# xingyizhou/CenterNet

Measured on AMD Instinct MI355X. Metric: images/sec whole-node, 512x512 ctdet, higher is better.
Workload: dtype f32s; 1 GPU; ctdet resdcn_18 512x512, batch 32 per GPU (BASELINE configs[1]), network + fused sigmoid/peak-NMS/top-K decode, K=100; global_batch=32, parallelism=image-sharded x1

## Files before the change

centernet_amd/csrc/cn_conv.hip:

```cpp
#include "cn_internal.h"
#include "cn_tuning.h"
#include <type_traits>

#ifndef CN_IGEMM_F32S_SETS
#define CN_IGEMM_F32S_SETS 1
#endif

namespace {

constexpr int NT = 256;
constexpr int BK = 32;
constexpr int LDT = BK + 4;

enum { A_DENSE = 0, A_STEM = 1, A_DCN = 2, A_DCN_PAD = 3 };
constexpr int STEM_KMAX = 512;

struct IgemmArgs {
    const void *x;
    const void *w;
    const float *bias;
    const float *scale;
    const float *shift;
    const void *residual;
    void *y;
// ... 596 lines not shown
            }
        }
    } else {
        const int OHW = a.OH * a.OW;
#pragma unroll
        for (int i = 0; i < MB; ++i) {
            const int off = rowoff[wm * TM + i * 32 + l31];
            const int b = off >= 0 ? off / OHW : 0;
            const int rem = off - b * OHW;
#pragma unroll
            for (int j = 0; j < NB; ++j) {
#pragma unroll
                for (int r = 0; r < 16; ++r) {
                    const int n = n0 + wn * TN + j * 32 + (r & 3) + 8 * (r >> 2) + 4 * lh;
                    if (off >= 0 && n < a.Cout) {
                        const float bs = a.bias ? a.bias[n] : 0.f;
                        const float sc = a.scale ? a.scale[n] : 1.f;
                        const float sf = a.shift ? a.shift[n] : 0.f;
                        float v = (acc[i][j][r] + bs) * sc + sf;
                        if (a.relu) v = fmaxf(v, 0.f);
                        reinterpret_cast<float *>(a.y)[((size_t)b * a.Cout + n) * OHW + rem] = v;
                    }
                }
            }
        }
    }
    if constexpr (SPLIT) {
        if (a.range) {
            if (!OUT_NCHW && !a.out_plain && a.ksplit <= 1) cn_rng_commit(a.range, 0, rng_out);
            if (DCN || a.in_plain) cn_rng_commit(a.range, 1, rng_in);
        }
    }
}

template <int BM, int BN, int WM, int AMODE, bool OUT_NCHW, int NBUF>
constexpr size_t igemm_lds_bytes()
{
    constexpr size_t tiles = (size_t)NBUF * (BM + BN) * LDT;
    constexpr size_t cs = OUT_NCHW ? 0 : (size_t)(BM / WM) * (BN + 4);
    return (tiles > cs ? tiles : cs) * 4 + BM * 4 +
           ((AMODE == A_DCN || AMODE == A_DCN_PAD) ? (size_t)9 * BM * (4 * 4 + 4 * 4 + 4) : 0) +
           (AMODE == A_STEM ? (size_t)STEM_KMAX * 8 : 0);
}

template <typename T, int BM, int BN, int WM, int WN, int AMODE, bool OUT_NCHW, int NBUF>
int launch_igemm_n(const IgemmArgs &a, hipStream_t st)
{
    constexpr size_t lds = igemm_lds_bytes<BM, BN, WM, AMODE, OUT_NCHW, NBUF>();
    CN_SET_MAX_LDS_ONCE((igemm_kernel<T, BM, BN, WM, WN, AMODE, OUT_NCHW, NBUF>), lds);
    dim3 grid(cn_cdiv(a.M, BM), cn_cdiv(a.Cout, BN), a.zparity ? 4 : (a.ksplit > 1 ? a.ksplit : 1));
    IgemmArgs b = a;
    b.xcd_swizzle = (grid.x >= 16 && cn_knobs.swz != 2 && (AMODE == A_DCN || AMODE == A_DCN_PAD || cn_knobs.swz == 1)) ? 1 : 0;
    b.setprio = cn_knobs.setprio;
    b.dbgskip = cn_knobs.dbgskip;
    hipLaunchKernelGGL((igemm_kernel<T, BM, BN, WM, WN, AMODE, OUT_NCHW, NBUF>), grid, dim3(NT),
                       lds, st, b);
    CN_CHECK_LAUNCH();
    return CN_OK;
}

template <int BM, int BN, int WM, int WN, int AMODE, bool OUT_NCHW>
int launch_igemm_h(const IgemmArgs &a, hipStream_t st)
{
    static_assert(AMODE != A_DCN && AMODE != A_DCN_PAD, "fp16 DCN is not built");
    if (!OUT_NCHW && AMODE == A_DENSE && a.stride == 1)
        return launch_igemm_n<_Float16, BM, BN, WM, WN, AMODE, OUT_NCHW, 1>(a, st);
    return launch_igemm_n<_Float16, BM, BN, WM, WN, AMODE, OUT_NCHW, 2>(a, st);
}

template <int BM, int BN, int WM, int WN, int AMODE, bool OUT_NCHW>
int launch_igemm_s(const IgemmArgs &a, hipStream_t st)
{
    static_assert(AMODE != A_STEM, "the stem stays on the fp32 kernel");
    if (!OUT_NCHW && a.stride == 1 && cn_knobs.nbuf != 2)
        return launch_igemm_n<cn_f32s, BM, BN, WM, WN, AMODE, OUT_NCHW, 1>(a, st);
    return launch_igemm_n<cn_f32s, BM, BN, WM, WN, AMODE, OUT_NCHW, 2>(a, st);
}

template <int BM, int BN, int WM, int WN, int AMODE, bool OUT_NCHW>
int launch_igemm(const IgemmArgs &a, hipStream_t st)
{
    int nbuf = cn_knobs.nbuf ? cn_knobs.nbuf : (a.stride == 1 ? 1 : 2);
    if (AMODE == A_STEM || OUT_NCHW) nbuf = 2;
    if (nbuf == 1) {
        if constexpr (AMODE != A_STEM && !OUT_NCHW)
            return launch_igemm_n<float, BM, BN, WM, WN, AMODE, OUT_NCHW, 1>(a, st);
    }
    return launch_igemm_n<float, BM, BN, WM, WN, AMODE, OUT_NCHW, 2>(a, st);
}

template <int BM, int BN, int WM, int WN, int AMODE, bool OUT_NCHW>
int launch_igemm_t(int dtype, const IgemmArgs &a, hipStream_t st)
{
    if constexpr (AMODE != A_STEM) {
        if (dtype == CN_DTYPE_F32S) return launch_igemm_s<BM, BN, WM, WN, AMODE, OUT_NCHW>(a, st);
    }
    if constexpr (AMODE == A_DENSE || AMODE == A_STEM) {
        if (dtype == CN_DTYPE_F16) return launch_igemm_h<BM, BN, WM, WN, AMODE, OUT_NCHW>(a, st);
    }
    return launch_igemm<BM, BN, WM, WN, AMODE, OUT_NCHW>(a, st);
}

inline int cout_class(int Cout) { return Cout > 64 ? 2 : (Cout > 32 ? 1 : 0); }
template <int AMODE, bool OUT_NCHW>
int igemm_dispatch(int dtype, int cls, bool bm64, const IgemmArgs &a, hipStream_t st)
{
    constexpr bool DCN = AMODE == A_DCN || AMODE == A_DCN_PAD;
// ... 488 lines not shown
{
    if (cn_knobs.nosplit || cn_knobs.dcn_split == 1) return 1;
    if (cn_knobs.dcn_split == 3 || cn_knobs.dcn_split == 9) return cn_knobs.dcn_split;
    const long wgs = (long)cn_cdiv(B * H * W, 64) * cn_cdiv(Cout, Cout > 64 ? 128 : 64);
    if (wgs >= 1024) return 1;
    return wgs * 3 >= 600 ? 3 : 9;
}

extern "C" size_t cn_dcn_v2_forward_nhwc_workspace_bytes(int B, int Cin, int H, int W, int Cout)
{
    if (B <= 0 || Cin <= 0 || H <= 0 || W <= 0 || Cout <= 0) return 0;
    const int s = dcn_ksplit(B, H, W, Cout);
    return s > 1 ? (size_t)(s > 8 ? s : 8) * B * H * W * round_up(Cout, 32) * sizeof(float) : 0;
}

extern "C" int cn_dcn_v2_forward_nhwc_f32(const float *input_nhwc, const float *weight_packed,
                                          const float *bias, const float *offset_mask_nhwc,
                                          int om_pitch, const float *scale, const float *shift,
                                          float *output_nhwc, int B, int Cin, int H, int W,
                                          int Cout, int mask_sigmoid, int relu, void *workspace,
                                          size_t workspace_bytes, void *stream)
{
    return cn_dcn_v2_forward_nhwc(input_nhwc, weight_packed, bias, offset_mask_nhwc, om_pitch, scale,
                                  shift, output_nhwc, Cout, B, Cin, H, W, Cout, mask_sigmoid, relu,
                                  CN_DTYPE_F32, 0, nullptr, workspace, workspace_bytes, stream);
}

extern "C" int cn_dcn_v2_forward_nhwc(const float *input_nhwc, const void *weight_packed,
                                      const float *bias, const float *offset_mask_nhwc,
                                      int om_pitch, const float *scale, const float *shift,
                                      void *output_nhwc, int out_pitch, int B, int Cin, int H,
                                      int W, int Cout, int mask_sigmoid, int relu, int dtype,
                                      int flags, const cn_f32s_ctl *ctl, void *workspace,
                                      size_t workspace_bytes, void *stream)
{
    if (!input_nhwc || !weight_packed || !offset_mask_nhwc || !output_nhwc) return CN_ERR_NULL;
    if (B <= 0 || Cin <= 0 || H <= 0 || W <= 0 || Cout <= 0 || out_pitch < Cout) return CN_ERR_SHAPE;
    if (om_pitch < 27) return CN_ERR_SHAPE;
    if ((Cin & 3) != 0) return CN_ERR_UNSUPPORTED;
    const bool f32s = (dtype == CN_DTYPE_F32S);
    if (dtype != CN_DTYPE_F32 && !f32s) return CN_ERR_UNSUPPORTED;
    if (f32s && !(flags & CN_CONV_Y_PLAIN) && (out_pitch & 31)) return CN_ERR_UNSUPPORTED;
    if (!cn_aligned16(input_nhwc) || !cn_aligned16(weight_packed)) return CN_ERR_ALIGN;
    if (f32s && !(flags & CN_CONV_Y_PLAIN) && !aligned128(output_nhwc)) return CN_ERR_ALIGN;
    if ((long)B * H * W * (long)(Cin > out_pitch ? Cin : out_pitch) >= (1L << 30)) return CN_ERR_UNSUPPORTED;
    if (f32s && cn_knobs.dcn_form != 1) {
        const bool forced = cn_knobs.dcn_form >= 2;
        const bool ws_ok = workspace && cn_aligned16(workspace) && !cn_knobs.nosplit;
        int ks = 1;
        int rc = CN_ERR_UNSUPPORTED;
        const long tiles128 = (long)B * (H / 8) * (W / 16);
        const bool team_auto = cn_knobs.dcn_form == 0 && tiles128 >= 64 &&
                               ((cn_knobs.dcn_team == 1 && Cout <= 64) || cn_knobs.dcn_team >= 2);
        const bool wide_auto = cn_knobs.dcn_form == 0 && cn_knobs.dcn_wide && tiles128 >= 64 && (Cout & 127) == 0 && !cn_knobs.dbgskip;
        DcnWinCall c = {};
        c.x = input_nhwc; c.w = weight_packed; c.bias = bias; c.om = offset_mask_nhwc; c.om_pitch = om_pitch;
        c.scale = scale; c.shift = shift; c.y = output_nhwc; c.out_pitch = out_pitch;
        c.out_plain = (flags & CN_CONV_Y_PLAIN) ? 1 : 0;
        c.B = B; c.Cin = Cin; c.H = H; c.W = W; c.Cout = Cout; c.mask_sigmoid = mask_sigmoid; c.relu = relu;
        c.x_mul = (ctl && ctl->x_mul != 0.f) ? ctl->x_mul : 1.f;
        c.range = ctl ? ctl->range : nullptr;
        c.dbg = cn_knobs.dbgskip;
        c.partial = ws_ok ? (float *)workspace : nullptr;
        c.partial_bytes = ws_ok ? workspace_bytes : 0;
        hipStream_t st = (hipStream_t)stream;
        if (cn_knobs.dcn_form == 6 || cn_knobs.dcn_form == 7 || wide_auto)
            rc = cn_dcn_wide_f32s(c, cn_knobs.dcn_form == 7 ? 4 : 0, &ks, st);
        if (rc == CN_ERR_UNSUPPORTED && (cn_knobs.dcn_form == 4 || cn_knobs.dcn_form == 5 || team_auto))
            rc = cn_dcn_team_f32s(c, cn_knobs.dcn_form == 5 ? 2 : ((team_auto && cn_knobs.dcn_team == 3) ? 1 : 0), &ks, st);
        if (rc == CN_ERR_UNSUPPORTED && cn_knobs.dcn_form < 4)
            rc = cn_dcn_window_f32s(c, forced ? 1 : 192, &ks, st);
        if (rc == CN_OK && ks > 1) {
            IgemmArgs r = {};
            r.bias = bias; r.scale = scale; r.shift = shift; r.residual = nullptr; r.y = output_nhwc;
            set_ctl(r, ctl);
            r.B = B; r.H = H; r.W = W; r.Ho = H; r.Wo = W; r.Cout = Cout; r.out_pitch = out_pitch;
            r.out_plain = (flags & CN_CONV_Y_PLAIN) ? 1 : 0;
            r.OH = H; r.OW = W; r.oy_mul = 1; r.oy_add = 0; r.ox_mul = 1; r.ox_add = 0;
            r.relu = relu; r.M = B * H * W; r.cout_pad = round_up(Cout, 32);
            r.ksplit = ks; r.partial = (float *)workspace;
            return launch_splitk_reduce(CN_DTYPE_F32S, r, 4096, (hipStream_t)stream);
        }
        if (rc != CN_ERR_UNSUPPORTED) return rc;
    }
    IgemmArgs a = {};
    a.x = input_nhwc; a.w = weight_packed; a.bias = bias; a.scale = scale; a.shift = shift;
    a.residual = nullptr; a.y = output_nhwc; a.om = offset_mask_nhwc; a.om_pitch = om_pitch;
    a.mask_sigmoid = mask_sigmoid;
    set_ctl(a, ctl);
    a.B = B; a.H = H; a.W = W; a.Cin = Cin; a.Ho = H; a.Wo = W; a.Cout = Cout;
    a.KH = 3; a.KW = 3; a.stride = 1; a.pad_h = 1; a.pad_w = 1; a.dil = 1;
    a.in_pitch = Cin; a.out_pitch = out_pitch;
    a.in_plain = 1;
    a.out_plain = (flags & CN_CONV_Y_PLAIN) ? 1 : 0;
    a.OH = H; a.OW = W; a.oy_mul = 1; a.oy_add = 0; a.ox_mul = 1; a.ox_add = 0;
    a.relu = relu;
    a.M = B * H * W;
    a.cin_pad = round_up(Cin, 32);
    a.cout_pad = round_up(Cout, 32);
    a.nchunk = a.cin_pad / 32;
    a.KT = 9 * a.nchunk;
    a.vec_out = ((Cout & 3) == 0 && (out_pitch & 3) == 0 && cn_aligned16(output_nhwc)) ? 1 : 0;
    hipStream_t st = (hipStream_t)stream;
    a.tile2d = (cn_knobs.dcn_tile2d && (W & 7) == 0 && (H % (Cout > 32 ? 8 : 16)) == 0) ? 1 : 0;
    a.ksplit = 1;
    if (Cout > 32) {
        const int want = dcn_ksplit(B, H, W, Cout);
        const size_t need = (size_t)want * a.M * a.cout_pad * sizeof(float);
        if (want > 1 && workspace && workspace_bytes >= need && cn_aligned16(workspace)) {
            a.ksplit = want;
            a.partial = (float *)workspace;
        }
    }
    const int rc = (Cin & 31) ? igemm_dispatch<A_DCN_PAD, false>(dtype, cout_class(Cout), false, a, st)
                              : igemm_dispatch<A_DCN, false>(dtype, cout_class(Cout), false, a, st);
// ... 144 lines not shown
```

centernet_amd/csrc/cn_heads_at.hip:

```cpp
#include "cn_common.h"
#include "cn_internal.h"

namespace {

constexpr int HA_NT = 256;
constexpr int HA_CELLS = 16;
constexpr int HA_CC = 64;
constexpr int HA_ROW = 9 * HA_CC;
constexpr int HA_MAXN = 768;
constexpr int HA_MAXJ = 17;
constexpr int HA_MAXOUT = 2 + 2 * HA_MAXJ + 2;
enum { HA_CTDET = 0, HA_POSE = 1, HA_DDD = 2 };
constexpr int HA_PF = 4;
constexpr int HA_MAXGROUPS = 5;
constexpr int HA_GROUP_HEADS = 3;
constexpr int HA_DDD_OUT = 16;

struct HeadsAtGroup {
    const cn_f32x4 *w1;
    const float *b1, *w2, *b2;
    int n_heads;
    int cout[HA_GROUP_HEADS];
    int col[HA_GROUP_HEADS];
    int voff[HA_GROUP_HEADS];
};

struct HeadsAtArgs {
    const char *feat;
    const float *scores;
    const int32_t *inds, *clses;
    const cn_f32x4 *w1;
    const float *b1;
    const float *w2;
    const float *b2;
    float *dets;
    float *vals;
    float mul;
    int H, W, Cin, pitch, K, hidden, n_heads, N;
    int c0, c1;
    int out;
    int J;
    HeadsAtGroup grp[HA_MAXGROUPS];
    int D;
    int vals_out;
    int raw_depth;
    int half_group;
};

__device__ __forceinline__ void ha_ctdet_row(const HeadsAtArgs &a, size_t row, int ind, const float *o)
{
    float *d = a.dets + row * 6;
    const float score = a.scores[row];
    const float cls = (float)a.clses[row];
    if (ind < 0) {
        const float nan = __builtin_nanf("");
        d[0] = nan; d[1] = nan; d[2] = nan; d[3] = nan; d[4] = score; d[5] = cls;
        if (a.vals)
            for (int v = 0; v < a.out; ++v) a.vals[row * a.out + v] = nan;
        return;
    }
    const int yi = ind / a.W, xi = ind - yi * a.W;
    float xs = (float)xi, ys = (float)yi;
    if (a.n_heads > 1) {
        xs = xs + o[2];
        ys = ys + o[3];
    } else {
        xs = xs + 0.5f;
        ys = ys + 0.5f;
    }
    const float w = o[0];
    const float h = o[1];
    d[0] = xs - w / 2;
    d[1] = ys - h / 2;
    d[2] = xs + w / 2;
    d[3] = ys + h / 2;
    d[4] = score;
    d[5] = cls;
    if (a.vals)
        for (int v = 0; v < a.out; ++v) a.vals[row * a.out + v] = o[v];
}

__device__ __forceinline__ float ha_pose_col(const HeadsAtArgs &a, size_t row, int ind, const float *o, int col)
{
    const int D = 5 + 2 * a.J + 1;
    if (col == 4) return a.scores[row];
    if (col == D - 1) return (float)a.clses[row];
    if (ind < 0) return __builtin_nanf("");
    const int yi = ind / a.W, xi = ind - yi * a.W;
    if (col >= 5) {
        const int v = col - 5;
        return o[2 + v] + (float)((v & 1) ? yi : xi);
    }
    const bool isy = col & 1;
    float c = (float)(isy ? yi : xi);
    if (a.n_heads > 2) c = c + o[2 + 2 * a.J + (isy ? 1 : 0)];
    else c = c + 0.5f;
    const float half = o[isy ? 1 : 0] / 2;
    return col < 2 ? c - half : c + half;
}

template <bool F32S, int CT, int NS, int TASK = HA_CTDET>
__global__ __launch_bounds__(HA_NT) void decode_heads_at_cells_kernel(const HeadsAtArgs a)
{
    constexpr int CG = HA_CELLS / CT;
    constexpr int TPC = HA_NT / CG;
    static_assert(TPC % 64 == 0, "the lanes of a wave read one cell's patch");
    constexpr int HROW = NS * TPC > HA_ROW ? NS * TPC : HA_ROW;
    static_assert(NS * TPC <= HA_MAXN && HA_CELLS * HROW * 4 <= 48 * 1024, "static LDS");
    __shared__ __attribute__((aligned(16))) float lds[HA_CELLS * HROW];
    __shared__ int s_ind[HA_CELLS];
    __shared__ float s_out[HA_CELLS * (TASK == HA_POSE ? HA_MAXOUT : TASK == HA_DDD ? HA_DDD_OUT : 4)];

    const int tid = threadIdx.x;
    const int b = blockIdx.y;
    const int k0 = blockIdx.x * HA_CELLS;
    const int ncell = min(HA_CELLS, a.K - k0);
    const int HW = a.H * a.W;
    int N = a.N, out = a.out, hc0 = a.c0, hc1 = a.c1;
    const cn_f32x4 *w1 = a.w1;
    const float *b1 = a.b1, *w2 = a.w2, *b2 = a.b2;
    if constexpr (TASK == HA_DDD) {
        const HeadsAtGroup &g = a.grp[blockIdx.z];
        N = g.n_heads * a.hidden;
        hc0 = g.cout[0];
        hc1 = g.cout[1];
        out = hc0 + hc1 + g.cout[2];
        w1 = g.w1; b1 = g.b1; w2 = g.w2; b2 = g.b2;
    }

    if (tid < HA_CELLS) {
        int ind = -1;
        if (tid < ncell) {
            ind = a.inds[(size_t)b * a.K + k0 + tid];
            if ((uint32_t)ind >= (uint32_t)HW) ind = -1;
        }
        s_ind[tid] = ind;
    }

    const int nl = tid % TPC, cg = tid / TPC;
    float acc[NS][CT];
#pragma unroll
    for (int s = 0; s < NS; ++s)
#pragma unroll
        for (int i = 0; i < CT; ++i) acc[s][i] = 0.f;

    size_t kq_base = 0;
    for (int c0 = 0; c0 < a.Cin; c0 += HA_CC) {
        const int cc = min(HA_CC, a.Cin - c0);
        const int cq = cc >> 2;
        __syncthreads();
        for (int i = tid; i < HA_CELLS * 9 * cq; i += HA_NT) {
            const int q = i % cq, r = i / cq;
            const int tap = r % 9, cell = r / 9;
            const int ind = s_ind[cell];
            cn_f32x4 v = {0.f, 0.f, 0.f, 0.f};
            if (ind >= 0) {
                const int y = ind / a.W + tap / 3 - 1, x = ind % a.W + tap % 3 - 1;
                if ((unsigned)y < (unsigned)a.H && (unsigned)x < (unsigned)a.W) {
                    const size_t pix = ((size_t)b * a.H + y) * a.W + x;
                    if (F32S) {
                        v = cn_load4_f32s(a.feat, pix, a.pitch, c0 + 4 * q);
                        v *= a.mul;
                    } else {
                        v = *reinterpret_cast<const cn_f32x4 *>(a.feat + (pix * (size_t)a.pitch + c0 + 4 * q) * 4);
                    }
                }
            }
            *reinterpret_cast<cn_f32x4 *>(&lds[cell * HA_ROW + tap * cc + 4 * q]) = v;
        }
        __syncthreads();

        const int nkq = 9 * cq;
        const cn_f32x4 *wq = w1 + kq_base * N;
        cn_f32x4 wn[HA_PF][NS];
#pragma unroll
        for (int p = 0; p < HA_PF; ++p)
#pragma unroll
            for (int s = 0; s < NS; ++s) {
                const int n = nl + s * TPC;
                wn[p][s] = n < N ? wq[(size_t)p * N + n] : cn_f32x4{0.f, 0.f, 0.f, 0.f};
            }
        for (int kq = 0; kq < nkq; kq += HA_PF) {
            cn_f32x4 wv[HA_PF][NS];
#pragma unroll
            for (int p = 0; p < HA_PF; ++p)
#pragma unroll
                for (int s = 0; s < NS; ++s) wv[p][s] = wn[p][s];
            if (kq + HA_PF < nkq) {
#pragma unroll
                for (int p = 0; p < HA_PF; ++p)
#pragma unroll
                    for (int s = 0; s < NS; ++s) {
                        const int n = nl + s * TPC;
                        if (n < N) wn[p][s] = wq[(size_t)(kq + HA_PF + p) * N + n];
                    }
            }
#pragma unroll
            for (int p = 0; p < HA_PF; ++p)
#pragma unroll
                for (int i = 0; i < CT; ++i) {
                    const cn_f32x4 pv = *reinterpret_cast<const cn_f32x4 *>(&lds[(i * CG + cg) * HA_ROW + 4 * (kq + p)]);
#pragma unroll
                    for (int s = 0; s < NS; ++s) {
                        float t = acc[s][i];
                        t = __builtin_fmaf(wv[p][s][0], pv[0], t);
                        t = __builtin_fmaf(wv[p][s][1], pv[1], t);
                        t = __builtin_fmaf(wv[p][s][2], pv[2], t);
                        t = __builtin_fmaf(wv[p][s][3], pv[3], t);
                        acc[s][i] = t;
                    }
                }
        }
        kq_base += (size_t)nkq;
    }

    __syncthreads();
#pragma unroll
    for (int s = 0; s < NS; ++s) {
        const int n = nl + s * TPC;
        if (n < N) {
            const float bias = b1[n];
#pragma unroll
            for (int i = 0; i < CT; ++i)
                lds[(i * CG + cg) * HROW + n] = __builtin_fmaxf(acc[s][i] + bias, 0.f);
        }
    }
    __syncthreads();

    const int nout = HA_CELLS * out;
    for (int o0 = 0; o0 < nout; o0 += HA_NT / 4) {
        const int o = o0 + (tid >> 2), sub = tid & 3;
        const bool live = o < nout;
        const int cell = o / out, r = o - cell * out;
        const int head = (r >= hc0) + (r >= hc0 + hc1);
        float sum = 0.f;
        if (live) {
            const float *w = w2 + (size_t)r * a.hidden;
            const float *h = &lds[cell * HROW + head * a.hidden];
            for (int c = sub; c < a.hidden; c += 4) sum = __builtin_fmaf(w[c], h[c], sum);
        }
        sum += __shfl_xor(sum, 1);
        sum += __shfl_xor(sum, 2);
        if (live && sub == 0) {
            if (b2) sum += b2[r];
            s_out[o] = sum;
        }
    }
    __syncthreads();

    if constexpr (TASK == HA_DDD) {
        const HeadsAtGroup &g = a.grp[blockIdx.z];
        const int D = a.D;
        for (int i = tid; i < ncell * out; i += HA_NT) {
            const int cell = i / out, r = i - cell * out;
            const int head = (r >= hc0) + (r >= hc0 + hc1);
            const int j = r - (head > 0 ? hc0 : 0) - (head > 1 ? hc1 : 0);
            const int col = (head == 0 ? g.col[0] : head == 1 ? g.col[1] : g.col[2]) + j;
            const int vcol = (head == 0 ? g.voff[0] : head == 1 ? g.voff[1] : g.voff[2]) + j;
            const size_t row = (size_t)b * a.K + k0 + cell;
            const int ind = s_ind[cell];
            const float raw = ind < 0 ? __builtin_nanf("") : s_out[i];
            float v = raw;
            if (ind >= 0) {
                if (col < 2) {
                    const int yi = ind / a.W, xi = ind - yi * a.W;
                    v = (float)(col ? yi : xi) + raw;
                } else if (col == 11 && a.raw_depth) {
                    v = 1.0f / (sigmoidf_ref(raw) + 1e-6f) - 1.0f;
                }
            }
            a.dets[row * D + col] = v;
            if (a.vals) a.vals[row * a.vals_out + vcol] = raw;
        }
        if (tid < ncell) {
            const size_t row = (size_t)b * a.K + k0 + tid;
            float *d = a.dets + row * D;
            if (blockIdx.z == 0) {
                d[2] = a.scores[row];
                d[D - 1] = (float)a.clses[row];
            }
            if ((int)blockIdx.z == a.half_group) {
                const int ind = s_ind[tid];
                const int yi = ind / a.W, xi = ind - yi * a.W;
                d[0] = ind < 0 ? __builtin_nanf("") : (float)xi + 0.5f;
                d[1] = ind < 0 ? __builtin_nanf("") : (float)yi + 0.5f;
            }
        }
    } else if (TASK == HA_CTDET) {
        if (tid < ncell) ha_ctdet_row(a, (size_t)b * a.K + k0 + tid, s_ind[tid], &s_out[tid * a.out]);
    } else {
        const int D = 5 + 2 * a.J + 1;
        for (int i = tid; i < ncell * D; i += HA_NT) {
            const int cell = i / D, col = i - cell * D;
            const size_t row = (size_t)b * a.K + k0 + cell;
            a.dets[row * D + col] = ha_pose_col(a, row, s_ind[cell], &s_out[cell * a.out], col);
        }
        if (a.vals)
            for (int i = tid; i < ncell * a.out; i += HA_NT) {
                const int cell = i / a.out;
                a.vals[((size_t)b * a.K + k0) * a.out + i] = s_ind[cell] < 0 ? __builtin_nanf("") : s_out[i];
            }
    }
}

__global__ void decode_pack_cell_w1_kernel(const float *__restrict__ w, float *__restrict__ out, int N, int Cin,
                                           size_t total)
{
    const size_t i = (size_t)blockIdx.x * blockDim.x + threadIdx.x;
    if (i >= total) return;
    const int e = (int)(i & 3);
    const int n = (int)((i >> 2) % N);
    const int k = (int)((i >> 2) / N) * 4 + e;
    const int chunk = k / (9 * HA_CC);
    const int c0 = chunk * HA_CC;
    const int cc = min(HA_CC, Cin - c0);
    const int r = k - chunk * 9 * HA_CC;
    const int tap = r / cc, ci = c0 + r % cc;
    out[i] = w[((size_t)n * Cin + ci) * 9 + tap];
}

}

extern "C" int cn_pack_cell_heads_w1(const float *w, float *out, int N, int Cin, void *stream)
{
    if (!w || !out) return CN_ERR_NULL;
    if (N <= 0 || Cin <= 0) return CN_ERR_SHAPE;
    if (N > HA_MAXN || (N & 63) || (Cin & 31)) return CN_ERR_UNSUPPORTED;
    if (!cn_aligned16(out)) return CN_ERR_ALIGN;
    const size_t total = (size_t)N * Cin * 9;
    hipLaunchKernelGGL(decode_pack_cell_w1_kernel, dim3((unsigned)((total + 255) / 256)), dim3(256), 0,
                       (hipStream_t)stream, w, out, N, Cin, total);
    CN_CHECK_LAUNCH();
    return CN_OK;
}

namespace {

template <int TASK>
void ha_launch(const HeadsAtArgs &a, int N, dim3 grid, bool s, hipStream_t st)
{
    const dim3 block(HA_NT);
#define HA_LAUNCH(CT, NS)                                                                                     \
    do {                                                                                                      \
        if (s) hipLaunchKernelGGL((decode_heads_at_cells_kernel<true, CT, NS, TASK>), grid, block, 0, st, a); \
        else hipLaunchKernelGGL((decode_heads_at_cells_kernel<false, CT, NS, TASK>), grid, block, 0, st, a);  \
    } while (0)
    if (N <= 64) {
        if constexpr (TASK != HA_POSE) HA_LAUNCH(4, 1);
    } else if (N <= 128) HA_LAUNCH(8, 1);
    else if (N <= 256) HA_LAUNCH(16, 1);
    else if (N <= 512) HA_LAUNCH(16, 2);
    else if constexpr (TASK != HA_CTDET) HA_LAUNCH(16, 3);
#undef HA_LAUNCH
}

template <class Limits, class Aligned>
int ha_prepare(HeadsAtArgs &a, const void *feat, int B, int H, int W, int Cin, int pitch, int dtype, float feat_mul,
               const float *scores, const int32_t *inds, const int32_t *clses, int K, int hidden, int n_heads,
               float *dets, float *head_vals, bool ptrs, bool counts, Limits limits, Aligned w1_aligned)
{
    if (!feat || !scores || !inds || !clses || !dets || !ptrs) return CN_ERR_NULL;
    if (B <= 0 || H <= 0 || W <= 0 || Cin <= 0 || K <= 0 || pitch < Cin || !counts) return CN_ERR_SHAPE;
    if (dtype != CN_DTYPE_F32S && dtype != CN_DTYPE_F32) return CN_ERR_UNSUPPORTED;
    if (hidden < 64 || hidden > 256 || (hidden & 63)) return CN_ERR_UNSUPPORTED;
    if (const int rc = limits()) return rc;
    if ((Cin & 31) || (pitch & 3) || (dtype == CN_DTYPE_F32S && (pitch & 31))) return CN_ERR_UNSUPPORTED;
    if ((long)H * W >= (1L << 31) || B > 65535) return CN_ERR_UNSUPPORTED;
    if (!cn_aligned16(feat) || !w1_aligned()) return CN_ERR_ALIGN;
    a.feat = (const char *)feat; a.scores = scores; a.inds = inds; a.clses = clses;
    a.dets = dets; a.vals = head_vals; a.mul = dtype == CN_DTYPE_F32S ? feat_mul : 1.f;
    a.H = H; a.W = W; a.Cin = Cin; a.pitch = pitch; a.K = K; a.hidden = hidden; a.n_heads = n_heads;
    return CN_OK;
}

template <int TASK>
int heads_at_cells(const void *feat, int B, int H, int W, int Cin, int pitch, int dtype, float feat_mul,
                   const float *scores, const int32_t *inds, const int32_t *clses, int K,
                   const float *w1_packed, const float *bias1, int hidden, int n_heads, int J, const float *w2,
                   const float *bias2, float *dets, float *head_vals, void *stream)
{
    constexpr int H0 = TASK == HA_POSE ? 2 : 1;
    HeadsAtArgs a;
    const int rc = ha_prepare(
        a, feat, B, H, W, Cin, pitch, dtype, feat_mul, scores, inds, clses, K, hidden, n_heads, dets, head_vals,
        w1_packed && bias1 && w2, true,
        [&] {
            if (n_heads < H0 || n_heads > H0 + 1) return CN_ERR_UNSUPPORTED;
            return TASK == HA_POSE && (J < 1 || J > HA_MAXJ) ? CN_ERR_UNSUPPORTED : CN_OK;
        },
        [&] { return cn_aligned16(w1_packed); });
    if (rc) return rc;
    a.w1 = (const cn_f32x4 *)w1_packed; a.b1 = bias1; a.w2 = w2; a.b2 = bias2;
    a.N = hidden * n_heads;
    a.J = J;
    a.c0 = 2;
    a.c1 = TASK == HA_POSE ? 2 * J : 2;
    a.out = TASK == HA_POSE ? 2 + 2 * J + (n_heads > 2 ? 2 : 0) : 2 * n_heads;
    ha_launch<TASK>(a, a.N, dim3((unsigned)cn_cdiv(K, HA_CELLS), (unsigned)B), dtype == CN_DTYPE_F32S,
                    (hipStream_t)stream);
    CN_CHECK_LAUNCH();
    return CN_OK;
}

}

extern "C" int cn_ctdet_heads_at_cells_f32(const void *feat, int B, int H, int W, int Cin, int pitch, int dtype,
                                           float feat_mul, const float *scores, const int32_t *inds,
                                           const int32_t *clses, int K, const float *w1_packed,
                                           const float *bias1, int hidden, int n_heads, const float *w2,
                                           const float *bias2, float *dets, float *head_vals, void *stream)
{
    return heads_at_cells<HA_CTDET>(feat, B, H, W, Cin, pitch, dtype, feat_mul, scores, inds, clses, K, w1_packed,
                                    bias1, hidden, n_heads, 0, w2, bias2, dets, head_vals, stream);
}

extern "C" int cn_multi_pose_heads_at_cells_f32(const void *feat, int B, int H, int W, int Cin, int pitch,
                                                int dtype, float feat_mul, const float *scores,
                                                const int32_t *inds, const int32_t *clses, int K,
                                                const float *w1_packed, const float *bias1, int hidden,
                                                int n_heads, int J, const float *w2, const float *bias2,
                                                float *dets, float *head_vals, void *stream)
{
    return heads_at_cells<HA_POSE>(feat, B, H, W, Cin, pitch, dtype, feat_mul, scores, inds, clses, K, w1_packed,
                                   bias1, hidden, n_heads, J, w2, bias2, dets, head_vals, stream);
}

extern "C" int cn_ddd_heads_at_cells_f32(const void *feat, int B, int H, int W, int Cin, int pitch, int dtype,
                                         float feat_mul, const float *scores, const int32_t *inds,
                                         const int32_t *clses, int K, int hidden, int n_groups,
                                         const cn_cell_head_group *groups, int has_wh, int has_reg, int flags,
                                         float *dets, float *head_vals, void *stream)
{
    const int n_heads = 3 + (has_wh ? 1 : 0) + (has_reg ? 1 : 0);
    int widest = 0;
    HeadsAtArgs a = {};
    const int rc = ha_prepare(
        a, feat, B, H, W, Cin, pitch, dtype, feat_mul, scores, inds, clses, K, hidden, n_heads, dets, head_vals,
        groups != nullptr, n_groups > 0,
        [&] {
            if (n_groups > HA_MAXGROUPS) return CN_ERR_UNSUPPORTED;
            int total = 0;
            for (int g = 0; g < n_groups; ++g) {
                const int n = groups[g].n_heads;
                if (n < 1 || n > HA_GROUP_HEADS || n * hidden > HA_MAXN) return CN_ERR_UNSUPPORTED;
                total += n;
                widest = n > widest ? n : widest;
            }
            if (total != n_heads) return CN_ERR_UNSUPPORTED;
            for (int g = 0; g < n_groups; ++g)
                if (!groups[g].w1_packed || !groups[g].bias1 || !groups[g].w2) return CN_ERR_NULL;
            return CN_OK;
        },
        [&] {
            for (int g = 0; g < n_groups; ++g)
                if (!cn_aligned16(groups[g].w1_packed)) return false;
            return true;
        });
    if (rc) return rc;
    const int couts[5] = {1, 8, 3, 2, 2};
    const int cols[5] = {11, 3, 12, has_wh ? 15 : 0, 0};
    a.D = has_wh ? 18 : 16;
    a.raw_depth = (flags & CN_DECODE_DDD_RAW_DEPTH) ? 1 : 0;
    a.half_group = has_reg ? -1 : 0;
    int head = 0, voff = 0;
    for (int g = 0; g < n_groups; ++g) {
        HeadsAtGroup &d = a.grp[g];
        d.w1 = (const cn_f32x4 *)groups[g].w1_packed;
        d.b1 = groups[g].bias1; d.w2 = groups[g].w2; d.b2 = groups[g].bias2;
        d.n_heads = groups[g].n_heads;
        for (int h = 0; h < d.n_heads; ++h, ++head) {
            const int t = head < 3 || has_wh ? head : 4;
            d.cout[h] = couts[t];
            d.col[h] = cols[t];
            d.voff[h] = voff;
            voff += couts[t];
        }
    }
    a.vals_out = voff;
    ha_launch<HA_DDD>(a, widest * hidden, dim3((unsigned)cn_cdiv(K, HA_CELLS), (unsigned)B, (unsigned)n_groups),
                      dtype == CN_DTYPE_F32S, (hipStream_t)stream);
    CN_CHECK_LAUNCH();
    return CN_OK;
}
```

centernet_amd/csrc/cn_tuning.h:

```cpp
#pragma once

struct CnTuning {
    int nbuf, narrow, bm, nosplit, nostem, swz, setprio, dbgskip, nohalo, stem_persist, dcn_split, bm256, waves8,
        split_min_chunks, split_max, stagger_pct, occ4, f32s_lds_weights, f32s_policy, dcn_tile2d, dcn_form,
        heads_remap, heads_reg, stem16s, c3p, c3p_stagger, c3p_knobs, c3p_heads, c3p_deconv, c3p_s2, dcn_team,
        dcn_team_wgs, dcn_team_stagger, offconv, offconv_teams1, dcn_wide, dcn_wide_wgs, stem_dbg, stem_stagger,
        dcn_wide_prefetch, proj, c3p_grid;
};
extern CnTuning cn_knobs;

struct CnTuningKey {
    int key;
    int CnTuning::*field;
    int def;
    int lo, hi;
    int n_also, also[4];
};

constexpr CnTuningKey CN_TUNING_KEYS[] = {
    {1, &CnTuning::nbuf, 0, 0, 2},
    {2, &CnTuning::narrow, 0, 0, 1},
    {3, nullptr, 0, 0, 0, 1, {64}},
    {4, &CnTuning::bm, 0, 0, 0, 2, {64, 128}},
    {5, &CnTuning::nosplit, 0, 0, 1},
    {6, &CnTuning::nostem, 0, 0, 1},
    {7, &CnTuning::swz, 0, 0, 2},
    {8, &CnTuning::setprio, 1, 0, 1},
    {9, &CnTuning::dbgskip, 0, 0, 2047},
    {10, &CnTuning::nohalo, 0, 0, 1},
    {11, nullptr, 0, 0, 0},
    {12, &CnTuning::stem_persist, 1, 0, 1},
    {13, &CnTuning::dcn_split, 0, 0, 1, 2, {3, 9}},
    {16, &CnTuning::split_min_chunks, 8, 1, 64},
    {17, &CnTuning::split_max, 16, 1, 64},
    {22, &CnTuning::dcn_tile2d, 1, 0, 1},
    {23, &CnTuning::dcn_form, 0, 0, 2, 4, {4, 5, 6, 7}},
    {27, &CnTuning::stem16s, 1, 0, 1},
    {14, &CnTuning::bm256, 0, 0, 3},
    {15, &CnTuning::waves8, 1, 0, 1},
    {18, &CnTuning::stagger_pct, 100, 0, 255},
    {19, &CnTuning::occ4, 0, 0, 2},
    {20, &CnTuning::f32s_lds_weights, 1, 0, 1},
    {21, &CnTuning::f32s_policy, 0, 0, 7},
    {24, &CnTuning::heads_remap, 1, 0, 3},
    {26, &CnTuning::heads_reg, 1, 0, 3},
    {28, &CnTuning::c3p, 1, 0, 7},
    {29, &CnTuning::c3p_stagger, 0, 0, 255},
    {30, &CnTuning::c3p_knobs, 2, 0, 255},
    {31, &CnTuning::c3p_heads, 1, 0, 1},
    {32, &CnTuning::c3p_deconv, 1, 0, 1},
    {33, &CnTuning::c3p_s2, 1, 0, 1},
    {47, &CnTuning::c3p_grid, 64, 1, 64},
    {36, &CnTuning::dcn_team, 3, 0, 3},
    {37, &CnTuning::dcn_team_wgs, 512, 1, 4096},
    {38, &CnTuning::dcn_team_stagger, 32, 0, 1024},
    {39, &CnTuning::offconv, 1, 0, 1},
    {40, &CnTuning::offconv_teams1, 768, 0, 1000000},
    {41, &CnTuning::dcn_wide, 1, 0, 1},
    {42, &CnTuning::dcn_wide_wgs, 256, 1, 4096},
    {45, &CnTuning::dcn_wide_prefetch, 1, 0, 1},
    {43, &CnTuning::stem_dbg, 0, 0, 31},
// ... 12 lines not shown
```

Baseline: 12440 img/s.

## Compute decode-time head MLPs at top-K cells with MFMA matrix kernel

Adds a matrix-core version of the heads-at-cells decode kernel. It gathers 32 cells' 3x3 patches into LDS and runs the first head layer with 32x32x2 f32 MFMA, optionally splitting K across waves and reducing through LDS. The W1 packing is changed to 32-row blocks to fit the MFMA fragment layout, and the old VALU path is kept behind a new debug bit. This targets the VALU-bound FMA loop in the post-network decode. The cost is heavier LDS use and more complex launch selection.

```diff
diff --git a/centernet_amd/csrc/cn_conv.hip b/centernet_amd/csrc/cn_conv.hip
--- a/centernet_amd/csrc/cn_conv.hip
+++ b/centernet_amd/csrc/cn_conv.hip
@@ -672,7 +672,7 @@
     IgemmArgs b = a;
     b.xcd_swizzle = (grid.x >= 16 && cn_knobs.swz != 2 && (AMODE == A_DCN || AMODE == A_DCN_PAD || cn_knobs.swz == 1)) ? 1 : 0;
     b.setprio = cn_knobs.setprio;
-    b.dbgskip = cn_knobs.dbgskip;
+    b.dbgskip = cn_knobs.dbgskip & CN_KNOB_ABLATION_BITS;
     hipLaunchKernelGGL((igemm_kernel<T, BM, BN, WM, WN, AMODE, OUT_NCHW, NBUF>), grid, dim3(NT),
                        lds, st, b);
     CN_CHECK_LAUNCH();
@@ -1267,7 +1267,7 @@
         const long tiles128 = (long)B * (H / 8) * (W / 16);
         const bool team_auto = cn_knobs.dcn_form == 0 && tiles128 >= 64 &&
                                ((cn_knobs.dcn_team == 1 && Cout <= 64) || cn_knobs.dcn_team >= 2);
-        const bool wide_auto = cn_knobs.dcn_form == 0 && cn_knobs.dcn_wide && tiles128 >= 64 && (Cout & 127) == 0 && !cn_knobs.dbgskip;
+        const bool wide_auto = cn_knobs.dcn_form == 0 && cn_knobs.dcn_wide && tiles128 >= 64 && (Cout & 127) == 0 && !(cn_knobs.dbgskip & CN_KNOB_ABLATION_BITS);
         DcnWinCall c = {};
         c.x = input_nhwc; c.w = weight_packed; c.bias = bias; c.om = offset_mask_nhwc; c.om_pitch = om_pitch;
         c.scale = scale; c.shift = shift; c.y = output_nhwc; c.out_pitch = out_pitch;
@@ -1275,7 +1275,7 @@
         c.B = B; c.Cin = Cin; c.H = H; c.W = W; c.Cout = Cout; c.mask_sigmoid = mask_sigmoid; c.relu = relu;
         c.x_mul = (ctl && ctl->x_mul != 0.f) ? ctl->x_mul : 1.f;
         c.range = ctl ? ctl->range : nullptr;
-        c.dbg = cn_knobs.dbgskip;
+        c.dbg = cn_knobs.dbgskip & CN_KNOB_ABLATION_BITS;
         c.partial = ws_ok ? (float *)workspace : nullptr;
         c.partial_bytes = ws_ok ? workspace_bytes : 0;
         hipStream_t st = (hipStream_t)stream;
diff --git a/centernet_amd/csrc/cn_heads_at.hip b/centernet_amd/csrc/cn_heads_at.hip
--- a/centernet_amd/csrc/cn_heads_at.hip
+++ b/centernet_amd/csrc/cn_heads_at.hip
@@ -1,5 +1,6 @@
 #include "cn_common.h"
 #include "cn_internal.h"
+#include "cn_tuning.h"
 
 namespace {
 
@@ -15,6 +16,17 @@
 constexpr int HA_MAXGROUPS = 5;
 constexpr int HA_GROUP_HEADS = 3;
 constexpr int HA_DDD_OUT = 16;
+constexpr int HM_NT = 512;
+constexpr int HM_CELLS = 32;
+constexpr int HM_PSTR = HM_CELLS + 1;
+constexpr int HM_PATCH = HA_ROW * HM_PSTR;
+constexpr int HM_W2 = 1024;
+constexpr int HM_PF = 18;
+
+__device__ __forceinline__ size_t ha_w1_at(int n, int kq, int nkq)
+{
+    return ((size_t)(n >> 5) * nkq + kq) * 32 + (n & 31);
+}
 
 struct HeadsAtGroup {
     const cn_f32x4 *w1;
@@ -99,6 +111,88 @@
     return col < 2 ? c - half : c + half;
 }
 
+template <int TASK, int NT, int CELLS>
+__device__ __forceinline__ void ha_tail(const HeadsAtArgs &a, const float *hid, int HROW, const int *s_ind,
+                                        float *s_out, const float *w2, const float *b2, int out, int hc0, int hc1,
+                                        int b, int k0, int ncell)
+{
+    const int tid = threadIdx.x;
+    const int nout = CELLS * out;
+    for (int o0 = 0; o0 < nout; o0 += NT / 4) {
+        const int o = o0 + (tid >> 2), sub = tid & 3;
+        const bool live = o < nout;
+        const int cell = o / out, r = o - cell * out;
+        const int head = (r >= hc0) + (r >= hc0 + hc1);
+        float sum = 0.f;
+        if (live) {
+            const float *w = w2 + (size_t)r * a.hidden;
+            const float *h = &hid[cell * HROW + head * a.hidden];
+            for (int c = sub; c < a.hidden; c += 4) sum = __builtin_fmaf(w[c], h[c], sum);
+        }
+        sum += __shfl_xor(sum, 1);
+        sum += __shfl_xor(sum, 2);
+        if (live && sub == 0) {
+            if (b2) sum += b2[r];
+            s_out[o] = sum;
+        }
+    }
+    __syncthreads();
+
+    if constexpr (TASK == HA_DDD) {
+        const HeadsAtGroup &g = a.grp[blockIdx.z];
+        const int D = a.D;
+        for (int i = tid; i < ncell * out; i += NT) {
+            const int cell = i / out, r = i - cell * out;
+            const int head = (r >= hc0) + (r >= hc0 + hc1);
+            const int j = r - (head > 0 ? hc0 : 0) - (head > 1 ? hc1 : 0);
+            const int col = (head == 0 ? g.col[0] : head == 1 ? g.col[1] : g.col[2]) + j;
+            const int vcol = (head == 0 ? g.voff[0] : head == 1 ? g.voff[1] : g.voff[2]) + j;
+            const size_t row = (size_t)b * a.K + k0 + cell;
+            const int ind = s_ind[cell];
+            const float raw = ind < 0 ? __builtin_nanf("") : s_out[i];
+            float v = raw;
+            if (ind >= 0) {
+                if (col < 2) {
+                    const int yi = ind / a.W, xi = ind - yi * a.W;
+                    v = (float)(col ? yi : xi) + raw;
+                } else if (col == 11 && a.raw_depth) {
+                    v = 1.0f / (sigmoidf_ref(raw) + 1e-6f) - 1.0f;
+                }
+            }
+            a.dets[row * D + col] = v;
+            if (a.vals) a.vals[row * a.vals_out + vcol] = raw;
+        }
+        if (tid < ncell) {
+            const size_t row = (size_t)b * a.K + k0 + tid;
+            float *d = a.dets + row * D;
+            if (blockIdx.z == 0) {
+                d[2] = a.scores[row];
+                d[D - 1] = (float)a.clses[row];
+            }
+            if ((int)blockIdx.z == a.half_group) {
+                const int ind = s_ind[tid];
+                const int yi = ind / a.W, xi = ind - yi * a.W;
+                d[0] = ind < 0 ? __builtin_nanf("") : (float)xi + 0.5f;
+                d[1] = ind < 0 ? __builtin_nanf("") : (float)yi + 0.5f;
+            }
+        }
+    } else if (TASK == HA_CTDET) {
+        if (tid < ncell) ha_ctdet_row(a, (size_t)b * a.K + k0 + tid, s_ind[tid], &s_out[tid * a.out]);
+    } else {
+        const int D = 5 + 2 * a.J + 1;
+        for (int i = tid; i < ncell * D; i += NT) {
+            const int cell = i / D, col = i - cell * D;
+            const size_t row = (size_t)b * a.K + k0 + cell;
+            a.dets[row * D + col] = ha_pose_col(a, row, s_ind[cell], &s_out[cell * a.out], col);
+        }
+        if (a.vals)
+            for (int i = tid; i < ncell * a.out; i += NT) {
+                const int cell = i / a.out;
+                a.vals[((size_t)b * a.K + k0) * a.out + i] = s_ind[cell] < 0 ? __builtin_nanf("") : s_out[i];
+            }
+    }
+}
+
 template <bool F32S, int CT, int NS, int TASK = HA_CTDET>
 __global__ __launch_bounds__(HA_NT) void decode_heads_at_cells_kernel(const HeadsAtArgs a)
 {
@@ -178,7 +272,7 @@
 #pragma unroll
             for (int s = 0; s < NS; ++s) {
                 const int n = nl + s * TPC;
-                wn[p][s] = n < N ? wq[(size_t)p * N + n] : cn_f32x4{0.f, 0.f, 0.f, 0.f};
+                wn[p][s] = n < N ? wq[ha_w1_at(n, p, nkq)] : cn_f32x4{0.f, 0.f, 0.f, 0.f};
             }
         for (int kq = 0; kq < nkq; kq += HA_PF) {
             cn_f32x4 wv[HA_PF][NS];
@@ -192,7 +286,7 @@
 #pragma unroll
                     for (int s = 0; s < NS; ++s) {
                         const int n = nl + s * TPC;
-                        if (n < N) wn[p][s] = wq[(size_t)(kq + HA_PF + p) * N + n];
+                        if (n < N) wn[p][s] = wq[ha_w1_at(n, kq + HA_PF + p, nkq)];
                     }
             }
 #pragma unroll
@@ -227,80 +321,204 @@
     }
     __syncthreads();
 
-    const int nout = HA_CELLS * out;
-    for (int o0 = 0; o0 < nout; o0 += HA_NT / 4) {
-        const int o = o0 + (tid >> 2), sub = tid & 3;
-        const bool live = o < nout;
-        const int cell = o / out, r = o - cell * out;
-        const int head = (r >= hc0) + (r >= hc0 + hc1);
-        float sum = 0.f;
-        if (live) {
-            const float *w = w2 + (size_t)r * a.hidden;
-            const float *h = &lds[cell * HROW + head * a.hidden];
-            for (int c = sub; c < a.hidden; c += 4) sum = __builtin_fmaf(w[c], h[c], sum);
-        }
-        sum += __shfl_xor(sum, 1);
-        sum += __shfl_xor(sum, 2);
-        if (live && sub == 0) {
-            if (b2) sum += b2[r];
-            s_out[o] = sum;
-        }
-    }
-    __syncthreads();
-
+    ha_tail<TASK, HA_NT, HA_CELLS>(a, lds, HROW, s_ind, s_out, w2, b2, out, hc0, hc1, b, k0, ncell);
+}
+
+template <bool F32S, int KS, int MPW, int TASK>
+__global__ __launch_bounds__(HM_NT) void decode_heads_at_cells_matrix_kernel(const HeadsAtArgs a)
+{
+    constexpr int MS = 8 / KS;
+    extern __shared__ __attribute__((aligned(16))) float lds[];
+    __shared__ int s_ind[HM_CELLS], s_y[HM_CELLS], s_x[HM_CELLS];
+    __shared__ float s_out[HM_CELLS * (TASK == HA_POSE ? HA_MAXOUT : TASK == HA_DDD ? HA_DDD_OUT : 4)];
+    __shared__ float s_b1[HA_MAXN], s_b2[HA_MAXOUT], s_w2[HM_W2];
+
+    const int tid = threadIdx.x, lane = tid & 63, wave = tid >> 6;
+    const int b = blockIdx.y;
+    const int k0 = blockIdx.x * HM_CELLS;
+    const int ncell = min(HM_CELLS, a.K - k0);
+    const int HW = a.H * a.W;
+    int N = a.N, out = a.out, hc0 = a.c0, hc1 = a.c1;
+    const cn_f32x4 *w1 = a.w1;
+    const float *b1 = a.b1, *w2 = a.w2, *b2 = a.b2;
     if constexpr (TASK == HA_DDD) {
         const HeadsAtGroup &g = a.grp[blockIdx.z];
-        const int D = a.D;
-        for (int i = tid; i < ncell * out; i += HA_NT) {
-            const int cell = i / out, r = i - cell * out;
-            const int head = (r >= hc0) + (r >= hc0 + hc1);
-            const int j = r - (head > 0 ? hc0 : 0) - (head > 1 ? hc1 : 0);
-            const int col = (head == 0 ? g.col[0] : head == 1 ? g.col[1] : g.col[2]) + j;
-            const int vcol = (head == 0 ? g.voff[0] : head == 1 ? g.voff[1] : g.voff[2]) + j;
-            const size_t row = (size_t)b * a.K + k0 + cell;
-            const int ind = s_ind[cell];
-            const float raw = ind < 0 ? __builtin_nanf("") : s_out[i];
-            float v = raw;
-            if (ind >= 0) {
-                if (col < 2) {
-                    const int yi = ind / a.W, xi = ind - yi * a.W;
-                    v = (float)(col ? yi : xi) + raw;
-                } else if (col == 11 && a.raw_depth) {
-                    v = 1.0f / (sigmoidf_ref(raw) + 1e-6f) - 1.0f;
-                }
-            }
-            a.dets[row * D + col] = v;
-            if (a.vals) a.vals[row * a.vals_out + vcol] = raw;
-        }
+        N = g.n_heads * a.hidden;
+        hc0 = g.cout[0];
+        hc1 = g.cout[1];
+        out = hc0 + hc1 + g.cout[2];
+        w1 = g.w1; b1 = g.b1; w2 = g.w2; b2 = g.b2;
+    }
+
+    if (tid < HM_CELLS) {
+        int ind = -1;
         if (tid < ncell) {
-            const size_t row = (size_t)b * a.K + k0 + tid;
-            float *d = a.dets + row * D;
-            if (blockIdx.z == 0) {
-                d[2] = a.scores[row];
-                d[D - 1] = (float)a.clses[row];
-            }
-            if ((int)blockIdx.z == a.half_group) {
-                const int ind = s_ind[tid];
-                const int yi = ind / a.W, xi = ind - yi * a.W;
-                d[0] = ind < 0 ? __builtin_nanf("") : (float)xi + 0.5f;
-                d[1] = ind < 0 ? __builtin_nanf("") : (float)yi + 0.5f;
-            }
-        }
-    } else if (TASK == HA_CTDET) {
-        if (tid < ncell) ha_ctdet_row(a, (size_t)b * a.K + k0 + tid, s_ind[tid], &s_out[tid * a.out]);
-    } else {
-        const int D = 5 + 2 * a.J + 1;
-        for (int i = tid; i < ncell * D; i += HA_NT) {
-            const int cell = i / D, col = i - cell * D;
-            const size_t row = (size_t)b * a.K + k0 + cell;
-            a.dets[row * D + col] = ha_pose_col(a, row, s_ind[cell], &s_out[cell * a.out], col);
-        }
-        if (a.vals)
-            for (int i = tid; i < ncell * a.out; i += HA_NT) {
-                const int cell = i / a.out;
-                a.vals[((size_t)b * a.K + k0) * a.out + i] = s_ind[cell] < 0 ? __builtin_nanf("") : s_out[i];
-            }
-    }
+            ind = a.inds[(size_t)b * a.K + k0 + tid];
+            if ((uint32_t)ind >= (uint32_t)HW) ind = -1;
+        }
+        s_ind[tid] = ind;
+        s_y[tid] = ind < 0 ? 0 : ind / a.W;
+        s_x[tid] = ind < 0 ? 0 : ind % a.W;
+    }
+    const bool w2_lds = out * a.hidden <= HM_W2;
+    for (int i = tid; i < N; i += HM_NT) s_b1[i] = b1[i];
+    if (b2 && tid < out) s_b2[tid] = b2[tid];
+    if (w2_lds)
+        for (int i = tid; i < out * a.hidden; i += HM_NT) s_w2[i] = w2[i];
+
+    const int ks = wave % KS, mslot = wave / KS;
+    int nact = 0;
+#pragma unroll
+    for (int j = 0; j < MPW; ++j) nact += (mslot + j * MS) * 32 < N;
+    cn_f32x16 acc[MPW];
+#pragma unroll
+    for (int j = 0; j < MPW; ++j)
+#pragma unroll
+        for (int v = 0; v < 16; ++v) acc[j][v] = 0.f;
+    const float *pb = lds + (lane >> 5) * 4 * HM_PSTR + (lane & 31);
+
+    size_t kq_base = 0;
+    for (int c0 = 0; c0 < a.Cin; c0 += HA_CC) {
+        const int cc = min(HA_CC, a.Cin - c0);
+        const int cq = cc >> 2, cqs = cc == HA_CC ? 4 : 3;
+        const int nkq = 9 * cq;
+        const int lpm = nkq / (2 * KS);
+        const int G = lpm / HM_PF;
+        const int s4_0 = ks * lpm;
+        const int total = nact * G;
+        const cn_f32x4 *wq = w1 + kq_base * N + lane;
+        auto frag = [&](int j, int g, int p) {
+            return wq + ((size_t)(mslot + j * MS) * nkq + 2 * (s4_0 + g * HM_PF + p)) * 32;
+        };
+        cn_f32x4 wn[HM_PF];
+        if (total > 0) {
+#pragma unroll
+            for (int p = 0; p < HM_PF; ++p) wn[p] = *frag(0, 0, p);
+        }
+
+        __syncthreads();
+        {
+            constexpr int NST = HM_CELLS * 9 * (HA_CC / 4) / HM_NT;
+            const int nitems = HM_CELLS * 9 * cq;
+            cn_f32x4 v[NST];
+#pragma unroll
+            for (int u = 0; u < NST; ++u) {
+                const int i = tid + u * HM_NT;
+                v[u] = cn_f32x4{0.f, 0.f, 0.f, 0.f};
+                if (i < nitems) {
+                    const int q = i & (cq - 1), r = i >> cqs;
+                    const int cell = r % HM_CELLS, tap = r / HM_CELLS;
+                    if (s_ind[cell] >= 0) {
+                        const int y = s_y[cell] + tap / 3 - 1, x = s_x[cell] + tap % 3 - 1;
+                        if ((unsigned)y < (unsigned)a.H && (unsigned)x < (unsigned)a.W) {
+                            const size_t pix = ((size_t)b * a.H + y) * a.W + x;
+                            if (F32S) {
+                                v[u] = cn_load4_f32s(a.feat, pix, a.pitch, c0 + 4 * q);
+                                v[u] *= a.mul;
+                            } else {
+                                v[u] = *reinterpret_cast<const cn_f32x4 *>(
+                                    a.feat + (pix * (size_t)a.pitch + c0 + 4 * q) * 4);
+                            }
+                        }
+                    }
+                }
+            }
+#pragma unroll
+            for (int u = 0; u < NST; ++u) {
+                const int i = tid + u * HM_NT;
+                if (i < nitems) {
+                    const int q = i & (cq - 1), r = i >> cqs;
+                    const int cell = r % HM_CELLS, tap = r / HM_CELLS;
+                    float *d = &lds[(tap * cc + 4 * q) * HM_PSTR + cell];
+                    d[0] = v[u][0];
+                    d[HM_PSTR] = v[u][1];
+                    d[2 * HM_PSTR] = v[u][2];
+                    d[3 * HM_PSTR] = v[u][3];
+                }
+            }
+        }
+        __syncthreads();
+
+        int flat = 0;
+#pragma unroll
+        for (int j = 0; j < MPW; ++j) {
+            for (int g = 0; j < nact && g < G; ++g) {
+                cn_f32x4 wv[HM_PF];
+#pragma unroll
+                for (int p = 0; p < HM_PF; ++p) wv[p] = wn[p];
+                if (++flat < total) {
+                    const int nj = flat / G, ng = flat - nj * G;
+#pragma unroll
+                    for (int p = 0; p < HM_PF; ++p) wn[p] = *frag(nj, ng, p);
+                }
+                const float *pg = pb + 8 * (s4_0 + g * HM_PF) * HM_PSTR;
+                float bq[4];
+#pragma unroll
+                for (int e = 0; e < 4; ++e) bq[e] = pg[e * HM_PSTR];
+#pragma unroll
+                for (int p = 0; p < HM_PF; ++p) {
+                    float bn[4];
+                    if (p + 1 < HM_PF) {
+#pragma unroll
+                        for (int e = 0; e < 4; ++e) bn[e] = pg[(8 * (p + 1) + e) * HM_PSTR];
+                    }
+                    __builtin_amdgcn_sched_barrier(0);
+#pragma unroll
+                    for (int e = 0; e < 4; ++e)
+                        acc[j] = __builtin_amdgcn_mfma_f32_32x32x2f32(wv[p][e], bq[e], acc[j], 0, 0, 0);
+                    __builtin_amdgcn_sched_barrier(0);
+                    if (p + 1 < HM_PF) {
+#pragma unroll
+                        for (int e = 0; e < 4; ++e) bq[e] = bn[e];
+                    }
+                }
+            }
+        }
+        kq_base += (size_t)nkq;
+    }
+
+    const int HROW = N + 1;
+    float *red = lds + ((HM_CELLS * HROW + 63) & ~63);
+    __syncthreads();
+    if constexpr (KS > 1) {
+        if (ks > 0) {
+#pragma unroll
+            for (int j = 0; j < MPW; ++j)
+                if (j < nact) {
+#pragma unroll
+                    for (int v = 0; v < 16; ++v)
+                        red[((((ks - 1) * MS + mslot) * MPW + j) * 16 + v) * 64 + lane] = acc[j][v];
+                }
+        }
+        __syncthreads();
+    }
+    if (ks == 0) {
+#pragma unroll
+        for (int j = 0; j < MPW; ++j)
+            if (j < nact) {
+                const int nb = (mslot + j * MS) * 32 + 4 * (lane >> 5);
+#pragma unroll
+                for (int v = 0; v < 16; ++v) {
+                    float t = acc[j][v];
+#pragma unroll
+                    for (int s = 1; s < KS; ++s) t += red[((((s - 1) * MS + mslot) * MPW + j) * 16 + v) * 64 + lane];
+                    const int n = nb + 8 * (v >> 2) + (v & 3);
+                    lds[(lane & 31) * HROW + n] = __builtin_fmaxf(t + s_b1[n], 0.f);
+                }
+            }
+    }
+    __syncthreads();
+
+    ha_tail<TASK, HM_NT, HM_CELLS>(a, lds, HROW, s_ind, s_out, w2_lds ? s_w2 : w2, b2 ? s_b2 : nullptr, out, hc0, hc1,
+                                   b, k0, ncell);
+}
+
+size_t hm_lds_bytes(int N, int KS, int MPW)
+{
+    const size_t hid = ((size_t)HM_CELLS * (N + 1) + 63) & ~(size_t)63;
+    const size_t red = KS > 1 ? (size_t)(KS - 1) * (8 / KS) * MPW * 16 * 64 : 0;
+    const size_t fl = hid + red > (size_t)HM_PATCH ? hid + red : (size_t)HM_PATCH;
+    return fl * sizeof(float);
 }
 
 __global__ void decode_pack_cell_w1_kernel(const float *__restrict__ w, float *__restrict__ out, int N, int Cin,
@@ -309,12 +527,16 @@
     const size_t i = (size_t)blockIdx.x * blockDim.x + threadIdx.x;
     if (i >= total) return;
     const int e = (int)(i & 3);
-    const int n = (int)((i >> 2) % N);
-    const int k = (int)((i >> 2) / N) * 4 + e;
-    const int chunk = k / (9 * HA_CC);
+    const size_t f = i >> 2;
+    const size_t per_chunk = (size_t)(9 * HA_CC / 4) * N;
+    const int chunk = (int)(f / per_chunk);
     const int c0 = chunk * HA_CC;
     const int cc = min(HA_CC, Cin - c0);
-    const int r = k - chunk * 9 * HA_CC;
+    const int nkq = 9 * cc / 4;
+    const int rem = (int)(f - chunk * per_chunk);
+    const int blk = rem / (nkq * 32), kq = rem / 32 % nkq;
+    const int n = blk * 32 + (rem & 31);
+    const int r = 4 * kq + e;
     const int tap = r / cc, ci = c0 + r % cc;
     out[i] = w[((size_t)n * Cin + ci) * 9 + tap];
 }
@@ -337,9 +559,32 @@
 namespace {
 
 template <int TASK>
-void ha_launch(const HeadsAtArgs &a, int N, dim3 grid, bool s, hipStream_t st)
-{
-    const dim3 block(HA_NT);
+void ha_launch(const HeadsAtArgs &a, int N, int groups, int B, bool s, hipStream_t st)
+{
+    if (!(cn_knobs.dbgskip & CN_KNOB_HEADS_AT_VALU) && (a.hidden == 64 || a.hidden == 256)) {
+        const dim3 grid((unsigned)cn_cdiv(a.K, HM_CELLS), (unsigned)B, (unsigned)groups), block(HM_NT);
+#define HM_LAUNCH(KS, MPW)                                                                              \
+    do {                                                                                                \
+        const size_t lds = hm_lds_bytes(N, KS, MPW);                                                    \
+        if (s) {                                                                                        \
+            CN_SET_MAX_LDS_ONCE((decode_heads_at_cells_matrix_kernel<true, KS, MPW, TASK>), 100 * 1024);  \
+            hipLaunchKernelGGL((decode_heads_at_cells_matrix_kernel<true, KS, MPW, TASK>), grid, block, lds, st, a);  \
+        } else {                                                                                        \
+            CN_SET_MAX_LDS_ONCE((decode_heads_at_cells_matrix_kernel<false, KS, MPW, TASK>), 100 * 1024); \
+            hipLaunchKernelGGL((decode_heads_at_cells_matrix_kernel<false, KS, MPW, TASK>), grid, block, lds, st, a); \
+        }                                                                                               \
+    } while (0)
+        if (a.hidden == 64) {
+            if (N <= 128) HM_LAUNCH(2, 1);
+            else HM_LAUNCH(2, 2);
+        } else if (N <= 256) {
+            if constexpr (TASK != HA_POSE) HM_LAUNCH(1, 1);
+        } else if (N <= 512) HM_LAUNCH(1, 2);
+        else if constexpr (TASK != HA_CTDET) HM_LAUNCH(1, 3);
+#undef HM_LAUNCH
+        return;
+    }
+    const dim3 grid((unsigned)cn_cdiv(a.K, HA_CELLS), (unsigned)B, (unsigned)groups), block(HA_NT);
 #define HA_LAUNCH(CT, NS)                                                                                     \
     do {                                                                                                      \
         if (s) hipLaunchKernelGGL((decode_heads_at_cells_kernel<true, CT, NS, TASK>), grid, block, 0, st, a); \
@@ -396,8 +641,7 @@
     a.c0 = 2;
     a.c1 = TASK == HA_POSE ? 2 * J : 2;
     a.out = TASK == HA_POSE ? 2 + 2 * J + (n_heads > 2 ? 2 : 0) : 2 * n_heads;
-    ha_launch<TASK>(a, a.N, dim3((unsigned)cn_cdiv(K, HA_CELLS), (unsigned)B), dtype == CN_DTYPE_F32S,
-                    (hipStream_t)stream);
+    ha_launch<TASK>(a, a.N, 1, B, dtype == CN_DTYPE_F32S, (hipStream_t)stream);
     CN_CHECK_LAUNCH();
     return CN_OK;
 }
@@ -477,8 +721,7 @@
         }
     }
     a.vals_out = voff;
-    ha_launch<HA_DDD>(a, widest * hidden, dim3((unsigned)cn_cdiv(K, HA_CELLS), (unsigned)B, (unsigned)n_groups),
-                      dtype == CN_DTYPE_F32S, (hipStream_t)stream);
+    ha_launch<HA_DDD>(a, widest * hidden, n_groups, B, dtype == CN_DTYPE_F32S, (hipStream_t)stream);
     CN_CHECK_LAUNCH();
     return CN_OK;
 }
diff --git a/centernet_amd/csrc/cn_tuning.h b/centernet_amd/csrc/cn_tuning.h
--- a/centernet_amd/csrc/cn_tuning.h
+++ b/centernet_amd/csrc/cn_tuning.h
@@ -7,6 +7,7 @@
         dcn_team_wgs, dcn_team_stagger, offconv, offconv_teams1, dcn_wide, dcn_wide_wgs, stem_dbg, stem_stagger,
         dcn_wide_prefetch, proj, c3p_grid;
 };
+constexpr int CN_KNOB_ABLATION_BITS = 1023, CN_KNOB_HEADS_AT_VALU = 1024;
 extern CnTuning cn_knobs;
 
 struct CnTuningKey {
```

Measured after the change: 12470 img/s, median of 2. About the same (+0.2%).
